# ortk95/planetmapper

Hardware: NVIDIA B200
Metric: full-backplane Mpix/s (FP64) + mapped-cube voxels/s at 1-8 B200 vs host CPU (higher is better)
Workload: dtype f64

## Files before the change

planetmapper_b200/csrc/backplane_kernels.cu:

```cuda
#include "pm_device.cuh"
#include "pm_kernels.h"

#include <cstdlib>

namespace pm {

constexpr int kPerThread = 4;
#ifndef PM_IMG_PARAM_CTAS
#define PM_IMG_PARAM_CTAS 4
#endif
constexpr int kImgParamCtas = PM_IMG_PARAM_CTAS;

__device__ __forceinline__ int slot(uint64_t mask, int k) { return __popcll(mask & (bit(k) - 1ull)); }

struct PlaneOffsets {
    int64_t byte_off[PM_N_PLANES];
    int64_t frame_stride;
};
static PlaneOffsets make_plane_offsets(uint64_t mask, int64_t plane_stride) {
    PlaneOffsets po;
    int slot = 0;
    for (int k = 0; k < PM_N_PLANES; k++) {
        po.byte_off[k] = (int64_t)slot * plane_stride * (int64_t)sizeof(double);
        if (mask & bit(k)) slot++;
    }
    po.frame_stride = (int64_t)slot * plane_stride;
    return po;
}

struct PlaneSink {
    char *base;
    const PlaneOffsets &po;
    __device__ __forceinline__ void put(int k, double v) const {
        __stcs(reinterpret_cast<double *>(base + po.byte_off[k]), v);
    }
};

template <bool kSky, uint64_t kFixedMask>
__device__ __forceinline__ void img_tile(const FrameD &fs, uint32_t tile, uint32_t nx, uint32_t npx, int per_thread,
                                         uint64_t mask, const PlaneOffsets &po, double *__restrict__ out) {
    uint32_t idx = tile * (uint32_t)(kBlock * per_thread) + threadIdx.x;
    uint32_t yi = idx / nx, xi = idx - yi * nx;
#pragma unroll 1
    for (int r = 0; r < per_thread && idx < npx; r++) {
        PlaneSink sink{reinterpret_cast<char *>(out + idx), po};
        image_pixel<kSky, kFixedMask>(fs, (double)xi, (double)yi, mask, sink);
        idx += kBlock;
        xi += kBlock;
        while (xi >= nx) {
            xi -= nx;
            yi++;
        }
    }
}

template <bool kSky, uint64_t kFixedMask>
__global__ void __launch_bounds__(kBlock, 4) backplanes_img_kernel(const PMFrame *__restrict__ frames, uint32_t nx,
                                                                   uint32_t npx, int per_thread, uint64_t mask,
                                                                   const __grid_constant__ PlaneOffsets po,
                                                                   double *__restrict__ out_all) {
    __shared__ FrameD fs;
    load_frame(fs, frames + blockIdx.y);
    img_tile<kSky, kFixedMask>(fs, blockIdx.x, nx, npx, per_thread, mask, po,
                               out_all + (int64_t)blockIdx.y * __popcll(mask) * npx);
}

__device__ __forceinline__ uint32_t centre_out_tile(uint32_t k, uint32_t n_tiles, uint32_t centre) {
    const uint32_t lo = centre, hi = n_tiles - 1u - centre;
    const uint32_t j = (k + 1u) >> 1;
    if (j <= min(lo, hi)) return (k & 1u) ? centre + j : centre - j;
    return lo < hi ? k : n_tiles - 1u - k;
}
template <bool kSky, uint64_t kFixedMask>
__global__ void __launch_bounds__(kBlock, kImgParamCtas) backplanes_img_param_kernel(
    const __grid_constant__ FrameD fs, uint32_t nx, uint32_t npx, int per_thread, uint32_t centre_tile, uint64_t mask,
    const __grid_constant__ PlaneOffsets po, double *__restrict__ out) {
    img_tile<kSky, kFixedMask>(fs, centre_out_tile(blockIdx.x, gridDim.x, centre_tile), nx, npx, per_thread, mask,
                               po, out);
}

template <bool kSky, bool kRingAll>
__global__ void __launch_bounds__(kBlock, 4) backplanes_points_param_kernel(const __grid_constant__ FrameD fs,
                                                                            const double *__restrict__ x_in,
                                                                            const double *__restrict__ y_in,
                                                                            int64_t n, uint64_t mask,
                                                                            const __grid_constant__ PlaneOffsets po,
                                                                            double *__restrict__ out) {
    const int64_t first = (int64_t)blockIdx.x * (kBlock * kPerThread) + threadIdx.x;
#pragma unroll 1
    for (int r = 0; r < kPerThread; r++) {
        const int64_t idx = first + r * kBlock;
        if (idx >= n) break;
        PlaneSink sink{reinterpret_cast<char *>(out + idx), po};
        image_point<kSky, kRingAll>(fs, __ldg(x_in + idx), __ldg(y_in + idx), mask, sink);
    }
}

constexpr uint64_t kXYMapMask = bit(PM_PIXEL_X) | bit(PM_PIXEL_Y);

template <uint64_t kFixedMask>
__device__ __forceinline__ void map_tile(const FrameD &fs, const double *__restrict__ lon_in,
                                         const double *__restrict__ lat_in, int64_t n, uint64_t mask,
                                         const PlaneOffsets &po, double *__restrict__ out) {
    const int64_t first = (int64_t)blockIdx.x * (kBlock * kPerThread) + threadIdx.x;
#pragma unroll 1
    for (int r = 0; r < kPerThread; r++) {
        const int64_t idx = first + r * kBlock;
        if (idx >= n) break;
        PlaneSink sink{reinterpret_cast<char *>(out + idx), po};
        map_cell<kFixedMask>(fs, __ldg(lon_in + idx), __ldg(lat_in + idx), mask, sink);
    }
}

template <uint64_t kFixedMask>
__global__ void __launch_bounds__(kBlock, 4) backplanes_map_kernel(const PMFrame *__restrict__ frame,
                                                                   const double *__restrict__ lon_in,
                                                                   const double *__restrict__ lat_in,
                                                                   int64_t n, uint64_t mask,
                                                                   const __grid_constant__ PlaneOffsets po,
                                                                   double *__restrict__ out) {
    __shared__ FrameD fs;
    load_frame(fs, frame + blockIdx.y);
    map_tile<kFixedMask>(fs, lon_in, lat_in, n, mask, po, out + (int64_t)blockIdx.y * po.frame_stride);
}

template <uint64_t kFixedMask>
__global__ void __launch_bounds__(kBlock, 4) backplanes_map_param_kernel(const __grid_constant__ FrameD fs,
// ... 148 lines not shown
    return (unsigned)(blocks < 1 ? 1 : blocks);
}

constexpr uint64_t kDefaultStackMask = kLonLatMask | kCentricMask | kIllumMask | kStateMask;

static int pick_per_thread(int64_t n, int64_t n_batches, int sm_count, int ctas_per_sm) {
    const int64_t tiles = ((n + kBlock - 1) / kBlock) * n_batches;
    const int64_t target = (int64_t)sm_count * ctas_per_sm * 3;
    int per = 16;
    while (per > 1 && tiles / per < target) per >>= 1;
    return per;
}

cudaError_t launch_backplanes_img(const PMFrame *frames, int n_frames, int nx, int ny, uint64_t mask,
                                  double *out, int sm_count, cudaStream_t st) {
    const int64_t npx = (int64_t)nx * ny;
    if (npx >= (1ll << 31)) return cudaErrorInvalidValue;
    const PlaneOffsets po = make_plane_offsets(mask, npx);
    static const int forced = tune_int("PM_IMG_PER_THREAD", 0);
    const int per = forced > 0 ? forced : pick_per_thread(npx, n_frames, sm_count, 4);
    const int64_t chunk = (int64_t)kBlock * per;
    dim3 grid((unsigned)((npx + chunk - 1) / chunk), n_frames);
    static const bool no_fixed = tune_int("PM_IMG_NO_FIXED_MASK", 0) != 0;
    if (mask == kDefaultStackMask && !no_fixed)
        backplanes_img_kernel<false, kDefaultStackMask><<<grid, kBlock, 0, st>>>(frames, (uint32_t)nx, (uint32_t)npx,
                                                                                   per, mask, po, out);
    else if (mask & kSkyMask)
        backplanes_img_kernel<true, 0><<<grid, kBlock, 0, st>>>(frames, (uint32_t)nx, (uint32_t)npx, per, mask, po, out);
    else
        backplanes_img_kernel<false, 0><<<grid, kBlock, 0, st>>>(frames, (uint32_t)nx, (uint32_t)npx, per, mask, po, out);
    count_launches(1);
    return cudaGetLastError();
}
cudaError_t launch_backplanes_img_host(const PMFrame *frame_host, int nx, int ny, uint64_t mask, double *out,
                                       int sm_count, cudaStream_t st) {
    const int64_t npx = (int64_t)nx * ny;
    if (npx >= (1ll << 31)) return cudaErrorInvalidValue;
    FrameD fs;
    load_frame_host(fs, frame_host);
    const PlaneOffsets po = make_plane_offsets(mask, npx);
    static const int forced = tune_int("PM_IMG_PER_THREAD", 0);
    const int per = forced > 0 ? forced : pick_per_thread(npx, 1, sm_count, kImgParamCtas);
    const int64_t chunk = (int64_t)kBlock * per;
    const int64_t n_tiles = (npx + chunk - 1) / chunk;
    dim3 grid((unsigned)n_tiles, 1);
    double cy = frame_host->y0 < 0.0 ? 0.0 : (frame_host->y0 > ny - 1.0 ? ny - 1.0 : frame_host->y0);
    double cx = frame_host->x0 < 0.0 ? 0.0 : (frame_host->x0 > nx - 1.0 ? nx - 1.0 : frame_host->x0);
    if (!(cy == cy) || !(cx == cx)) cy = cx = 0.0;
    int64_t ct = ((int64_t)cy * nx + (int64_t)cx) / chunk;
    static const bool linear = tune_int("PM_IMG_ORDER", 1) == 0;
    if (linear) ct = 0;
    const uint32_t centre = (uint32_t)(ct < 0 ? 0 : (ct >= n_tiles ? n_tiles - 1 : ct));
    if (mask == kDefaultStackMask)
        backplanes_img_param_kernel<false, kDefaultStackMask><<<grid, kBlock, 0, st>>>(
            fs, (uint32_t)nx, (uint32_t)npx, per, centre, mask, po, out);
    else if (mask & kSkyMask)
        backplanes_img_param_kernel<true, 0><<<grid, kBlock, 0, st>>>(fs, (uint32_t)nx, (uint32_t)npx, per, centre, mask,
                                                                       po, out);
    else
        backplanes_img_param_kernel<false, 0><<<grid, kBlock, 0, st>>>(fs, (uint32_t)nx, (uint32_t)npx, per, centre, mask,
                                                                        po, out);
    count_launches(1);
    return cudaGetLastError();
}
cudaError_t launch_backplanes_points_host(const PMFrame *frame_host, const double *x, const double *y, int64_t n,
                                          uint64_t mask, uint32_t flags, double *out, cudaStream_t st) {
    FrameD fs;
    load_frame_host(fs, frame_host);
    const PlaneOffsets po = make_plane_offsets(mask, n);
    const unsigned grid = chunks_for(n);
    if (!(mask & kSkyMask))
        backplanes_points_param_kernel<false, false><<<grid, kBlock, 0, st>>>(fs, x, y, n, mask, po, out);
    else if (flags & PM_FLAG_RING_ALL)
        backplanes_points_param_kernel<true, true><<<grid, kBlock, 0, st>>>(fs, x, y, n, mask, po, out);
    else
        backplanes_points_param_kernel<true, false><<<grid, kBlock, 0, st>>>(fs, x, y, n, mask, po, out);
    count_launches(1);
    return cudaGetLastError();
}
cudaError_t launch_backplanes_map(const PMFrame *frames, int n_frames, const double *lon, const double *lat,
                                  int64_t n, uint64_t mask, double *out, int sm_count, cudaStream_t st) {
    (void)sm_count;
    const dim3 grid(chunks_for(n), (unsigned)n_frames);
    const PlaneOffsets po = make_plane_offsets(mask, n);
    if (mask == kXYMapMask)
        backplanes_map_kernel<kXYMapMask><<<grid, kBlock, 0, st>>>(frames, lon, lat, n, mask, po, out);
    else
        backplanes_map_kernel<0><<<grid, kBlock, 0, st>>>(frames, lon, lat, n, mask, po, out);
    count_launches(1);
    return cudaGetLastError();
}
cudaError_t launch_backplanes_map_host(const PMFrame *frame_host, const double *lon, const double *lat, int64_t n,
                                       uint64_t mask, double *out, int sm_count, cudaStream_t st) {
    (void)sm_count;
    FrameD fs;
    load_frame_host(fs, frame_host);
    const PlaneOffsets po = make_plane_offsets(mask, n);
    if (mask == kXYMapMask)
        backplanes_map_param_kernel<kXYMapMask><<<chunks_for(n), kBlock, 0, st>>>(fs, lon, lat, n, mask, po, out);
    else
        backplanes_map_param_kernel<0><<<chunks_for(n), kBlock, 0, st>>>(fs, lon, lat, n, mask, po, out);
    count_launches(1);
    return cudaGetLastError();
}
cudaError_t launch_xy2lonlat(const PMFrame *frame, const double *x, const double *y, int64_t n, double *lon,
                             double *lat, unsigned long long *n_missed, int sm_count, cudaStream_t st) {
    (void)sm_count;
    xy2lonlat_kernel<<<chunks_for(n), kBlock, 0, st>>>(frame, x, y, n, lon, lat, n_missed);
    count_launches(1);
// ... 39 lines not shown
```

planetmapper_b200/csrc/pm_device.cuh:

```cuda
#pragma once

#include "../../include/pm_b200.h"
#include "pm_math.cuh"

namespace pm {

struct V3 {
    double x, y, z;
};

PM_HD V3 mk(double x, double y, double z) { return V3{x, y, z}; }
PM_HD V3 operator+(V3 a, V3 b) { return mk(a.x + b.x, a.y + b.y, a.z + b.z); }
PM_HD V3 operator-(V3 a, V3 b) { return mk(a.x - b.x, a.y - b.y, a.z - b.z); }
PM_HD V3 operator-(V3 a) { return mk(-a.x, -a.y, -a.z); }
PM_HD V3 operator*(double s, V3 a) { return mk(s * a.x, s * a.y, s * a.z); }
PM_HD double dot(V3 a, V3 b) { return fma(a.x, b.x, fma(a.y, b.y, a.z * b.z)); }
PM_HD V3 cross(V3 a, V3 b) {
    return mk(fma(a.y, b.z, -a.z * b.y), fma(a.z, b.x, -a.x * b.z), fma(a.x, b.y, -a.y * b.x));
}
PM_HD V3 mul3(V3 a, const double *s) { return mk(a.x * s[0], a.y * s[1], a.z * s[2]); }
PM_HD V3 axpy(double s, V3 b, V3 a) { return mk(fma(s, b.x, a.x), fma(s, b.y, a.y), fma(s, b.z, a.z)); }
PM_HD double norm(V3 a) { return fast_sqrt_lite(dot(a, a)); }
PM_HD V3 ld3(const double *p) { return mk(p[0], p[1], p[2]); }
PM_HD bool finite3(V3 a) { return fabs(a.x) < INFINITY && fabs(a.y) < INFINITY && fabs(a.z) < INFINITY; }
PM_HD V3 mxv(const double *m, V3 v) {
    return mk(fma(m[0], v.x, fma(m[1], v.y, m[2] * v.z)), fma(m[3], v.x, fma(m[4], v.y, m[5] * v.z)),
              fma(m[6], v.x, fma(m[7], v.y, m[8] * v.z)));
}
PM_HD V3 mtxv(const double *m, V3 v) {
    return mk(fma(m[0], v.x, fma(m[3], v.y, m[6] * v.z)), fma(m[1], v.x, fma(m[4], v.y, m[7] * v.z)),
              fma(m[2], v.x, fma(m[5], v.y, m[8] * v.z)));
}
PM_HD_NOINLINE double pymod360_slow(double a) {
    double r = ::fmod(a, 360.0);
    if (r != 0.0 && r < 0.0) r += 360.0;
    return r;
}
PM_HD double pymod360(double a) { return (a >= 0.0 && a < 360.0) ? a : pymod360_slow(a); }

struct FrameD {
    PMFrame f;
    double inv_c;
    double inv_r[3];
    double nw[3];
    double k[3];
    double wn;
    double rp;
    double e2, ep2;
    double inv_omf2;
    double omf;
    double P0b[3], VTb[3], ATb[3], VOb[3], S0b[3], VSb[3];
    double G[9];
    double y0[3];
    double y0m2;
    double As[6];
    double inv_kmpa;
    int biaxial;
    int pad_;
};

constexpr int kDeriveItems = 13;

PM_HD double ex_mul(double a, double b) {
#ifdef __CUDA_ARCH__
    return __dmul_rn(a, b);
#else
    return a * b;
#endif
}
PM_HD double ex_add(double a, double b) {
#ifdef __CUDA_ARCH__
    return __dadd_rn(a, b);
#else
    return a + b;
#endif
}
PM_HD double ex_div(double a, double b) {
#ifdef __CUDA_ARCH__
    return __ddiv_rn(a, b);
#else
    return a / b;
#endif
}
PM_HD double ex_sqrt(double a) {
#ifdef __CUDA_ARCH__
    return __dsqrt_rn(a);
#else
    return ::sqrt(a);
#endif
}
PM_HD double ex_dot3(double a0, double b0, double a1, double b1, double a2, double b2) {
    return ex_add(ex_add(ex_mul(a0, b0), ex_mul(a1, b1)), ex_mul(a2, b2));
}

PM_HD void derive_frame_item(FrameD &s, int item) {
    const PMFrame &f = s.f;
    if (item >= 3 && item <= 8) {
        const double *src = item == 3 ? f.P0 : item == 4 ? f.VT : item == 5 ? f.AT : item == 6 ? f.VO : item == 7 ? f.S0 : f.VS;
        double *dst = item == 3 ? s.P0b : item == 4 ? s.VTb : item == 5 ? s.ATb : item == 6 ? s.VOb : item == 7 ? s.S0b : s.VSb;
        for (int r = 0; r < 3; r++)
            dst[r] = ex_dot3(f.R0[3 * r], src[0], f.R0[3 * r + 1], src[1], f.R0[3 * r + 2], src[2]);
        if (item == 3) {
            for (int r = 0; r < 3; r++) s.y0[r] = ex_mul(-dst[r], ex_div(1.0, f.radii[r]));
            s.y0m2 = fma(s.y0[0], s.y0[0], fma(s.y0[1], s.y0[1], ex_mul(s.y0[2], s.y0[2])));
        }
    } else if (item >= 9 && item <= 11) {
        const int r = item - 9;
        for (int c = 0; c < 3; c++)
            s.G[3 * r + c] = ex_dot3(f.R0[3 * r], f.M[3 * c], f.R0[3 * r + 1], f.M[3 * c + 1], f.R0[3 * r + 2], f.M[3 * c + 2]);
    } else if (item == 12) {
        const double sc = kRpd / 3600.0;
        for (int c = 0; c < 3; c++) {
            s.As[c] = -ex_mul(f.A[c], sc);
            s.As[3 + c] = ex_mul(f.A[3 + c], sc);
        }
        s.inv_kmpa = ex_div(1.0, f.km_per_arcsec);
    } else if (item == 0) {
        s.inv_c = ex_div(1.0, f.clight);
        const double w2 = ex_dot3(f.omega[0], f.omega[0], f.omega[1], f.omega[1], f.omega[2], f.omega[2]);
        const double wn = ex_sqrt(w2);
        s.wn = wn;
        s.k[0] = wn > 0.0 ? ex_div(f.omega[0], wn) : 0.0;
        s.k[1] = wn > 0.0 ? ex_div(f.omega[1], wn) : 0.0;
        s.k[2] = wn > 0.0 ? ex_div(f.omega[2], wn) : 0.0;
    } else if (item == 1) {
        const double a = f.radii[0], b = f.radii[1], c = f.radii[2];
        s.inv_r[0] = ex_div(1.0, a);
        s.inv_r[1] = ex_div(1.0, b);
        s.inv_r[2] = ex_div(1.0, c);
        const double m = fmin(a, fmin(b, c));
        const double ma = ex_div(m, a), mb = ex_div(m, b), mc = ex_div(m, c);
        s.nw[0] = ex_mul(ma, ma);
        s.nw[1] = ex_mul(mb, mb);
        s.nw[2] = ex_mul(mc, mc);
    } else if (item == 2) {
        const double rp = ex_add(f.re, -ex_mul(f.f, f.re));
        const double re2 = ex_mul(f.re, f.re), rp2 = ex_mul(rp, rp);
        const double omf = ex_add(1.0, -f.f);
        s.rp = rp;
        s.e2 = ex_add(1.0, -ex_div(rp2, re2));
        s.ep2 = ex_add(ex_div(re2, rp2), -1.0);
        s.omf = omf;
        s.inv_omf2 = ex_div(1.0, ex_mul(omf, omf));
        s.biaxial = (f.radii[0] == f.radii[1]) && (f.re == f.radii[0]) && (fabs(rp - f.radii[2]) <= 4e-16 * f.radii[2]);
        s.pad_ = 0;
    }
}

#ifdef __CUDACC__
__device__ __forceinline__ void load_frame(FrameD &s, const PMFrame *__restrict__ g) {
    const double *src = reinterpret_cast<const double *>(g);
    double *dst = reinterpret_cast<double *>(&s.f);
    for (int i = threadIdx.x; i < PM_FRAME_NDOUBLES; i += blockDim.x) dst[i] = __ldg(src + i);
    __syncthreads();
    const int w = threadIdx.x >> 5, l = threadIdx.x & 31;
    int item = -1;
    if (blockDim.x >= 128) {
        if (w == 0 && l < 6) item = 3 + l;
        else if (w == 1 && l < 4) item = 9 + l;
        else if (w == 2 && l < 2) item = l;
        else if (w == 3 && l == 0) item = 2;
    } else if (threadIdx.x < kDeriveItems) {
        item = threadIdx.x;
    }
    if (item >= 0) derive_frame_item(s, item);
    __syncthreads();
}
#endif
inline void load_frame_host(FrameD &s, const PMFrame *g) {
    s.f = *g;
    for (int i = 0; i < kDeriveItems; i++) derive_frame_item(s, i);
}

#ifndef PM_GRAZING_COS2
#define PM_GRAZING_COS2 3.0e-3
#endif
constexpr double kGrazingCos2 = PM_GRAZING_COS2;

// ... 38 lines not shown
    const V3 t = mk(fma(k.x, ku, -u.x), fma(k.y, ku, -u.y), fma(k.z, ku, -u.z));
    return axpy(r.omc, t, axpy(r.s, kxu, u));
}
PM_HD V3 spin_bwd(const FrameD &fs, Rot r, V3 u) { return spin_bwd_c(fs, r, u, cross(ld3(fs.k), u)); }
PM_HD V3 to_body(const FrameD &fs, Rot r, V3 v) { return spin_fwd(fs, r, mxv(fs.f.R0, v)); }
PM_HD V3 from_body(const FrameD &fs, Rot r, V3 u) { return mtxv(fs.f.R0, spin_bwd(fs, r, u)); }
PM_HD V3 target_pos_b(const FrameD &fs, double dt) {
    const double h = 0.5 * dt * dt;
    return mk(fma(fs.ATb[0], h, fma(fs.VTb[0], dt, fs.P0b[0])), fma(fs.ATb[1], h, fma(fs.VTb[1], dt, fs.P0b[1])),
              fma(fs.ATb[2], h, fma(fs.VTb[2], dt, fs.P0b[2])));
}

PM_HD void recrad_angles(V3 v, double &ra, double &dec) {
    dec = fast_atan2_xpos(v.z, fast_sqrt(fma(v.x, v.x, v.y * v.y)));
    double lon = fast_atan2(v.y, v.x);
    if (lon < 0.0) lon += kTwoPi;
    ra = lon;
}
PM_HD V3 radrec1(double ra, double dec) {
    double sr, cr, sd, cd;
    sincos_full(ra, sr, cr);
    sincos_full(dec, sd, cd);
    return mk(cr * cd, sr * cd, sd);
}
PM_HD double vsep(V3 a, V3 b) { return fast_atan2_ypos(norm(cross(a, b)), dot(a, b)); }

struct RayHit {
    V3 pp;
    double ixx;
    double a;
    double t;
    double cos2;
};
PM_HD bool surfpt_y(const FrameD &fs, V3 y, double ym2, V3 u, V3 &p, RayHit &hit) {
    const V3 x = mul3(u, fs.inv_r);
    const double xx = dot(x, x), yx = dot(y, x);
    if (!(xx > 0.0)) return false;
    const double ixx = fast_rcp(xx);
    const double a = -(yx * ixx);
    const V3 pp = axpy(a, x, y);
    const double pm2 = dot(pp, pp);
    if (!(pm2 < INFINITY)) return false;
    hit.pp = pp;
    hit.ixx = ixx;
    hit.a = a;
    hit.cos2 = 1.0 - pm2;
    double h;
    if (ym2 > 1.0) {
        if (pm2 > 1.0) return false;
        if (yx > 0.0) return false;
        h = -fast_sqrt_lite((1.0 - pm2) * ixx);
    } else if (ym2 == 1.0) {
        h = -a;
    } else {
        h = fast_sqrt_lite(fmax(0.0, 1.0 - pm2) * ixx);
    }
    hit.t = a + h;
    p = mul3(axpy(h, x, pp), fs.f.radii);
    return true;
}
PM_HD bool surfpt(const FrameD &fs, V3 o, V3 u, V3 &p, RayHit &hit) {
    const V3 y = mul3(o, fs.inv_r);
    return surfpt_y(fs, y, dot(y, y), u, p, hit);
}

struct Intercept {
    V3 p;
    V3 u;
    Rot r;
    double dt;
    double L;
    double lt;
};

PM_HD_NOINLINE bool sincpt_converge(const FrameD &fs, V3 u0, double &dt, V3 &p, double &range) {
    const PMFrame &f = fs.f;
    for (int it = 0; it < 8; it++) {
        const Rot r = make_rot(fs, dt);
        const V3 o = spin_fwd(fs, r, -target_pos_b(fs, dt));
        RayHit hit;
        if (!surfpt(fs, o, spin_fwd(fs, r, u0), p, hit)) return false;
        range = hit.t;
        const double t = dt + f.t_ref;
        const double t_new = f.et - hit.t * fs.inv_c;
        if (!(fabs(t_new - t) > 1.0e-17 * fabs(t_new))) break;
        dt = t_new - f.t_ref;
    }
    return true;
}

PM_HD bool sincpt(const FrameD &fs, V3 u0, Intercept &it) {
    const PMFrame &f = fs.f;
    V3 p1, p2;
    RayHit h1, h2;
    if (!surfpt_y(fs, ld3(fs.y0), fs.y0m2, u0, p1, h1)) return false;
    const double lt1 = h1.t * fs.inv_c;

    const double dt1 = (f.et - lt1) - f.t_ref;
    const Rot r1 = make_rot(fs, dt1);
    if (!surfpt(fs, spin_fwd(fs, r1, -target_pos_b(fs, dt1)), spin_fwd(fs, r1, u0), p2, h2)) return false;
    const double lt2 = h2.t * fs.inv_c;

    double dt = (f.et - lt2) - f.t_ref;
    V3 p;
    double L;
    if (fabs(dt1) > PM_T(kPixC)[kPixDt1Min] && h2.cos2 > PM_T(kPixC)[kPixGrazing]) {
        const double lam = fast_div_lite(dt - dt1, dt1 - (dt - dt1));
        dt = fma(lam, dt1, dt1) + f.t_ref;
        dt -= f.t_ref;
        const V3 pps = axpy(lam, h2.pp - h1.pp, h2.pp);
        const double hs = fast_sqrt_lite(fmax(1.0 - dot(pps, pps), 0.0) * fma(lam, h2.ixx - h1.ixx, h2.ixx));
        L = fma(lam, h2.a - h1.a, h2.a) - hs;
        it.r = make_rot(fs, dt);
        it.u = spin_fwd(fs, it.r, u0);
        p = axpy(-hs, it.u, mul3(pps, fs.f.radii));
    } else {
        double dt_c = dt, L_c;
        V3 p_c;
        if (!sincpt_converge(fs, u0, dt_c, p_c, L_c)) return false;
        dt = dt_c;
        p = p_c;
        L = L_c;
        it.r = make_rot(fs, dt);
        it.u = spin_fwd(fs, it.r, u0);
    }
    it.p = p;
    it.dt = dt;
    it.L = L;
    it.lt = L * fs.inv_c;
    return true;
}

PM_HD void geodetic_general(const FrameD &fs, double rho, double z, double &lat, double &alt) {
    const PMFrame &f = fs.f;
    if (f.f == 0.0) {
        lat = fast_atan2_xpos(z, rho);
        alt = fast_sqrt(fma(rho, rho, z * z)) - f.re;
        return;
    }
    double sb = f.re * z, cb = fs.rp * rho;
    double n = fast_rsqrt(fma(sb, sb, cb * cb) + sqrt_guard());
    sb *= n;
    cb *= n;
    double num = z, den = rho;
#pragma unroll 1
    for (int i = 0; i < 8; i++) {
        num = fma(fs.ep2 * fs.rp, sb * sb * sb, z);
        den = fma(-fs.e2 * f.re, cb * cb * cb, rho);
        double nsb = fs.omf * num, ncb = den;
        n = fast_rsqrt(fma(nsb, nsb, ncb * ncb) + sqrt_guard());
        nsb *= n;
        ncb *= n;
        const double change = fabs(nsb - sb) + fabs(ncb - cb);
        sb = nsb;
        cb = ncb;
        if (change <= 4.0e-16) break;
    }
// ... 79 lines not shown
PM_HD_NOINLINE double doppler_factor_closed(double beta) { return fast_sqrt(fast_div(1.0 + beta, 1.0 - beta)); }
PM_HD_NOINLINE double light_time_rate_closed(double a, double b, double c) { return fast_div(a - b, c + a); }
PM_HD double doppler_factor(const FrameD &fs, double rv) {
    const double beta = rv * fs.inv_c;
    if (fabs(beta) < PM_T(kPixC)[kPixBetaMax])
        return fma(beta, fma(beta, fma(beta, fma(beta, fma(beta, 0.375, 0.375), 0.5), 0.5), 1.0), 1.0);
    return doppler_factor_closed(beta);
}

PM_HD double radial_velocity(const FrameD &fs, double a, double b) {
    const double ac = a * fs.inv_c;
    double dlt = (a - b) * fs.inv_c * fma(ac, ac - 1.0, 1.0);
    if (!(fabs(ac) < PM_T(kPixC)[kPixBetaMax])) dlt = light_time_rate_closed(a, b, fs.f.clight);
    return fma(-dlt, a, a) - b;
}

struct Illum {
    double phase, incdnc, emissn, azimuth;
};
PM_HD void illum_angles(V3 n, V3 s, V3 e, bool want_az, Illum &out) {
    const V3 cse = cross(s, e), cns = cross(n, s), cne = cross(n, e);
    const double dse = dot(s, e), dns = dot(n, s), dne = dot(n, e);
    const double mns = norm(cns), mne = norm(cne);
    out.phase = fast_atan2_ypos(norm(cse), dse);
    out.incdnc = fast_atan2_ypos(mns, dns);
    out.emissn = fast_atan2_ypos(mne, dne);
    if (want_az) {
        const double nn = dot(n, n);
        const double a = fma(dse, nn, -dne * dns);
        out.azimuth = fast_atan2_ypos(fast_sqrt_pos(nn) * fabs(dot(n, cse)), -a);
    }
}

PM_HD void illum_at(const FrameD &fs, V3 p, V3 p0 , V3 e, Rot r, double dt, bool want_az,
                    Illum &out) {
    const PMFrame &f = fs.f;
    const double h = 0.5 * dt * dt;
    const V3 base = mk(fs.S0b[0] - fma(fs.ATb[0], h, fma(fs.VTb[0], dt, p0.x)),
                       fs.S0b[1] - fma(fs.ATb[1], h, fma(fs.VTb[1], dt, p0.y)),
                       fs.S0b[2] - fma(fs.ATb[2], h, fma(fs.VTb[2], dt, p0.z)));
    const V3 VSb = ld3(fs.VSb);
    V3 sv = axpy(dt, VSb, base);
    const double lts = fast_sqrt_pos(dot(sv, sv)) * fs.inv_c;
    sv = axpy(dt - (lts - f.lts0), VSb, base);
    const V3 s_b = spin_fwd(fs, r, sv);
    const V3 n = mul3(p, fs.nw);
    illum_angles(n, s_b, e, want_az, out);
}

struct PointGeom {
    V3 p0;
    V3 X0;
    Rot r;
    double dt, L, lt;
};
PM_HD void point_geom(const FrameD &fs, V3 p, PointGeom &g) {
    const PMFrame &f = fs.f;
    double lt = norm(ld3(fs.P0b) + p) * fs.inv_c;
#pragma unroll 1
    for (int pass = 0; pass < 2; pass++) {
        const double dt = (f.et - lt) - f.t_ref;
        const Rot r = make_rot(fs, dt);
        const V3 p0 = spin_bwd(fs, r, p);
        const V3 X0 = target_pos_b(fs, dt) + p0;
        const double L = norm(X0);
        lt = L * fs.inv_c;
        g.p0 = p0;
        g.X0 = X0;
        g.r = r;
        g.dt = dt;
        g.L = L;
        g.lt = lt;
    }
}
PM_HD double point_rv(const FrameD &fs, V3 p, const PointGeom &g) {
    const double iL = fast_rcp(g.L);
    const V3 ph0 = iL * g.X0;
    const V3 vt = axpy(g.dt, ld3(fs.ATb), ld3(fs.VTb));
// ... 58 lines not shown

PM_HD void limb_coordinates(const FrameD &fs, V3 ov, double &lon_deg, double &lat_deg, double &dist) {
    const PMFrame &f = fs.f;
    lon_deg = lat_deg = dist = NAN;
    const double n2 = dot(ov, ov);
    if (!(n2 > 0.0)) return;
    const V3 u = fast_rsqrt(n2) * ov;
    const V3 P0 = ld3(f.P0);
    const V3 pn = dot(P0, u) * u;
    const double near_dist = norm(P0 - pn);
    const V3 tv = obsvec2targvec(fs, pn);
    const V3 x = mul3(tv, fs.inv_r);
    const double xn2 = dot(x, x);
    if (!(xn2 > 0.0)) return;
    const V3 sp = fast_rsqrt(xn2) * tv;
    double lon, lat, alt;
    recpgr(fs, sp, fs.biaxial != 0, lon, lat, alt);
    lon_deg = lon * kDpr;
    lat_deg = lat * kDpr;
    dist = near_dist - norm(sp);
}

PM_HD constexpr uint64_t bit(int k) { return 1ull << k; }
constexpr uint64_t kKmMask = bit(PM_KM_X) | bit(PM_KM_Y) | bit(PM_ANGULAR_X) | bit(PM_ANGULAR_Y);
constexpr uint64_t kLonLatMask = bit(PM_LON_GRAPHIC) | bit(PM_LAT_GRAPHIC) | bit(PM_LOCAL_SOLAR_TIME);
constexpr uint64_t kCentricMask = bit(PM_LON_CENTRIC) | bit(PM_LAT_CENTRIC);
constexpr uint64_t kIllumMask = bit(PM_PHASE) | bit(PM_INCIDENCE) | bit(PM_EMISSION) | bit(PM_AZIMUTH);
constexpr uint64_t kStateMask = bit(PM_DISTANCE) | bit(PM_RADIAL_VELOCITY) | bit(PM_DOPPLER);
constexpr uint64_t kLimbMask = bit(PM_LIMB_DISTANCE) | bit(PM_LIMB_LON_GRAPHIC) | bit(PM_LIMB_LAT_GRAPHIC);
constexpr uint64_t kRingMask = bit(PM_RING_RADIUS) | bit(PM_RING_LON_GRAPHIC) | bit(PM_RING_DISTANCE);
constexpr uint64_t kSurfMask = kLonLatMask | kCentricMask | kIllumMask | kStateMask | kRingMask;
constexpr uint64_t kSkyMask = bit(PM_RA) | bit(PM_DEC) | kKmMask | kLimbMask | kRingMask;

template <bool kSky, uint64_t kFixedMask = 0, bool kRingAll = false, class Sink>
PM_HD void image_pixel(const FrameD &fs, double x, double y, uint64_t mask_in, Sink &out) {
    const PMFrame &f = fs.f;
    const double nan = NAN;
    const uint64_t mask = kFixedMask ? kFixedMask : (kSky ? mask_in : (mask_in & ~kSkyMask));
    if (mask & bit(PM_PIXEL_X)) out.put(PM_PIXEL_X, x);
    if (mask & bit(PM_PIXEL_Y)) out.put(PM_PIXEL_Y, y);

    const double dx = x - f.x0, dy = y - f.y0;
    const bool try_disc = (mask & kSurfMask) && !(f.optimize_speed != 0.0 && fma(dx, dx, dy * dy) > f.r_cut2);
    V3 v = mk(nan, nan, nan);
    if (try_disc || (kSky && (mask & kSkyMask))) v = xy2ray_local(fs, x, y);
    V3 d2 = mk(nan, nan, nan);
    if (kSky && (mask & kSkyMask)) {
        const V3 d = mtxv(f.M, v);
        double ra, dec;
        recrad_angles(d, ra, dec);
        const double ra_deg = ra * kDpr, dec_deg = dec * kDpr;
        if (mask & bit(PM_RA)) out.put(PM_RA, ra_deg);
        if (mask & bit(PM_DEC)) out.put(PM_DEC, dec_deg);
        if (mask & (kKmMask | kLimbMask | kRingMask)) d2 = radrec1(ra_deg * kRpd, dec_deg * kRpd);
        if (mask & kKmMask) {
            double ax, ay;
            obsvec2angular(f, d2, ax, ay);
            const double kx = fma(f.ang2km[0], ax, f.ang2km[1] * ay);
            const double ky = fma(f.ang2km[2], ax, f.ang2km[3] * ay);
            if (mask & bit(PM_KM_X)) out.put(PM_KM_X, kx);
            if (mask & bit(PM_KM_Y)) out.put(PM_KM_Y, ky);
            if (mask & bit(PM_ANGULAR_X)) out.put(PM_ANGULAR_X, fast_div(kx, f.km_per_arcsec));
            if (mask & bit(PM_ANGULAR_Y)) out.put(PM_ANGULAR_Y, fast_div(ky, f.km_per_arcsec));
        }
    }

    bool on_disc = false;
    Intercept it;
    const V3 u0 = mxv(fs.G, v);
    if (try_disc) on_disc = sincpt(fs, u0, it);

    double v_dist = nan;
    if (on_disc) {
        const V3 p = it.p;
        if (mask & (kLonLatMask | kCentricMask)) {
            const double rho = fast_sqrt_lite(fma(p.x, p.x, p.y * p.y));
            const double lon_e = fast_atan2(p.y, p.x);
            if (mask & kLonLatMask) {
                double l = f.lon_sign * lon_e;
                if (l < 0.0) l += kTwoPi;
                const double v_lon = l * kDpr;
                double lat, alt;
                if (fs.biaxial) {
                    lat = fast_atan2_xpos(p.z * fs.inv_omf2, rho);
                } else {
                    geodetic_general(fs, rho, p.z, lat, alt);
                }
                if (mask & bit(PM_LON_GRAPHIC)) out.put(PM_LON_GRAPHIC, v_lon);
                if (mask & bit(PM_LAT_GRAPHIC)) out.put(PM_LAT_GRAPHIC, lat * kDpr);
                if (mask & bit(PM_LOCAL_SOLAR_TIME)) out.put(PM_LOCAL_SOLAR_TIME, local_solar_time(f, v_lon));
            }
            if (mask & bit(PM_LON_CENTRIC)) out.put(PM_LON_CENTRIC, lon_e * kDpr);
            if (mask & bit(PM_LAT_CENTRIC)) out.put(PM_LAT_CENTRIC, fast_atan2_xpos(p.z, rho) * kDpr);
        }
        if (mask & (kIllumMask | kStateMask | kRingMask)) {
            const V3 kxp = cross(ld3(fs.k), p);
            const V3 p0 = spin_bwd_c(fs, it.r, p, kxp);
            if (mask & kIllumMask) {
                Illum il;
                illum_at(fs, p, p0, -it.u, it.r, it.dt, (mask & bit(PM_AZIMUTH)) != 0, il);
                if (mask & bit(PM_PHASE)) out.put(PM_PHASE, il.phase * kDpr);
                if (mask & bit(PM_INCIDENCE)) out.put(PM_INCIDENCE, il.incdnc * kDpr);
                if (mask & bit(PM_EMISSION)) out.put(PM_EMISSION, il.emissn * kDpr);
                if (mask & bit(PM_AZIMUTH)) out.put(PM_AZIMUTH, il.azimuth * kDpr);
            }
            v_dist = it.lt * f.clight;
            if (mask & bit(PM_DISTANCE)) out.put(PM_DISTANCE, v_dist);
            if (mask & (bit(PM_RADIAL_VELOCITY) | bit(PM_DOPPLER))) {
                const V3 vt = axpy(it.dt, ld3(fs.ATb), ld3(fs.VTb));
                const double a = fma(fs.wn, dot(kxp, it.u), dot(vt, u0));
                const double b = dot(ld3(fs.VOb), u0);
                const double rv = radial_velocity(fs, a, b);
                if (mask & bit(PM_RADIAL_VELOCITY)) out.put(PM_RADIAL_VELOCITY, rv);
                if (mask & bit(PM_DOPPLER)) out.put(PM_DOPPLER, doppler_factor(fs, rv));
            }
        }
    } else {
        const uint64_t m = mask & (kLonLatMask | kCentricMask | kIllumMask | kStateMask);
#pragma unroll
        for (int k = 0; k <= PM_DOPPLER; k++)
            if ((kLonLatMask | kCentricMask | kIllumMask | kStateMask) & bit(k))
                if (m & bit(k)) out.put(k, nan);
    }

    if (kSky && (mask & kLimbMask)) {
        double llon, llat, ldist;
        limb_coordinates(fs, d2, llon, llat, ldist);
        if (mask & bit(PM_LIMB_DISTANCE)) out.put(PM_LIMB_DISTANCE, ldist);
        if (mask & bit(PM_LIMB_LON_GRAPHIC)) out.put(PM_LIMB_LON_GRAPHIC, llon);
        if (mask & bit(PM_LIMB_LAT_GRAPHIC)) out.put(PM_LIMB_LAT_GRAPHIC, llat);
    }
    if (kSky && (mask & kRingMask)) {
        double rad, rl, rd;
        ring_coordinates(fs, d2, rad, rl, rd);
        if (!kRingAll && rd > v_dist) rad = rl = rd = nan;
        if (mask & bit(PM_RING_RADIUS)) out.put(PM_RING_RADIUS, rad);
        if (mask & bit(PM_RING_LON_GRAPHIC)) out.put(PM_RING_LON_GRAPHIC, rl);
        if (mask & bit(PM_RING_DISTANCE)) out.put(PM_RING_DISTANCE, rd);
    }
}

template <bool kSky, bool kRingAll, class Sink>
PM_HD void image_point(const FrameD &fs, double x, double y, uint64_t mask_in, Sink &out) {
    if (fabs(x) < INFINITY && fabs(y) < INFINITY) {
        image_pixel<kSky, 0, kRingAll>(fs, x, y, mask_in, out);
        return;
    }
#pragma unroll 1
    for (int k = 0; k < PM_N_PLANES; k++)
        if (mask_in & bit(k)) out.put(k, k == PM_PIXEL_X ? x : (k == PM_PIXEL_Y ? y : (double)NAN));
}

template <uint64_t kFixedMask = 0, class Sink>
PM_HD void map_cell(const FrameD &fs, double lon_deg, double lat_deg, uint64_t mask_in, Sink &out) {
    const uint64_t mask = kFixedMask ? kFixedMask : mask_in;
    const PMFrame &f = fs.f;
    const double nan = NAN;
    const double lonm = (fabs(lon_deg) < INFINITY) ? pymod360(lon_deg) : nan;
    const double latm = (fabs(lat_deg) < INFINITY) ? lat_deg : nan;
    if (mask & bit(PM_LON_GRAPHIC)) out.put(PM_LON_GRAPHIC, lonm);
    if (mask & bit(PM_LAT_GRAPHIC)) out.put(PM_LAT_GRAPHIC, latm);
    const bool lon_ok = lonm == lonm;
    const bool ok = lon_ok && (latm == latm);
    if (mask & bit(PM_LOCAL_SOLAR_TIME))
        out.put(PM_LOCAL_SOLAR_TIME, lon_ok ? local_solar_time(f, lonm) : nan);

    double v_clon = nan, v_clat = nan, v_g = nan, v_i = nan, v_e = nan, v_az = nan, v_dist = nan, v_rv = nan,
           v_dop = nan, v_ra = nan, v_dec = nan, v_x = nan, v_y = nan, v_kx = nan, v_ky = nan, v_ax = nan,
           v_ay = nan;
    double limb_lon = nan, limb_lat = nan, limb_dist = nan, ring_rad = nan, ring_lon = nan, ring_dist = nan;
    if (ok) {
        const V3 tv = pgrrec0(fs, lonm * kRpd, latm * kRpd);
        if (mask & kCentricMask) {
            double lo, la;
            reclat_angles(tv, lo, la);
            v_clon = lo * kDpr;
            v_clat = la * kDpr;
        }
// ... 246 lines not shown
```

Measured before the change: 30270.

## Add spin-symmetric fast path skipping body rotations in surface intercept

Adds a per-frame flag, computed when frame data is derived, marking bodies that are axisymmetric about the spin axis with negligible light-time rotation shift. For such frames, templated kernel variants skip the rotation of the observer position and ray direction inside the light-time intercept iterations. They reuse the ray-scaled direction and its reciprocal across both surface solves, and compute illumination in the unrotated frame without rotating the sun vector or the intercept point back. This cuts FP64 arithmetic per pixel, at the cost of extra kernel instantiations and code size, and results within the stated tolerance of the shift threshold may differ slightly.

New measurement: 32750 (median of 6 runs). +8.2%, better.

```diff
diff --git a/planetmapper_b200/csrc/backplane_kernels.cu b/planetmapper_b200/csrc/backplane_kernels.cu
--- a/planetmapper_b200/csrc/backplane_kernels.cu
+++ b/planetmapper_b200/csrc/backplane_kernels.cu
@@ -36,7 +36,7 @@
     }
 };
 
-template <bool kSky, uint64_t kFixedMask>
+template <bool kSky, uint64_t kFixedMask, bool kSpinSym>
 __device__ __forceinline__ void img_tile(const FrameD &fs, uint32_t tile, uint32_t nx, uint32_t npx, int per_thread,
                                          uint64_t mask, const PlaneOffsets &po, double *__restrict__ out) {
     uint32_t idx = tile * (uint32_t)(kBlock * per_thread) + threadIdx.x;
@@ -44,7 +44,7 @@
 #pragma unroll 1
     for (int r = 0; r < per_thread && idx < npx; r++) {
         PlaneSink sink{reinterpret_cast<char *>(out + idx), po};
-        image_pixel<kSky, kFixedMask>(fs, (double)xi, (double)yi, mask, sink);
+        image_pixel<kSky, kFixedMask, false, kSpinSym>(fs, (double)xi, (double)yi, mask, sink);
         idx += kBlock;
         xi += kBlock;
         while (xi >= nx) {
@@ -61,8 +61,11 @@
                                                                    double *__restrict__ out_all) {
     __shared__ FrameD fs;
     load_frame(fs, frames + blockIdx.y);
-    img_tile<kSky, kFixedMask>(fs, blockIdx.x, nx, npx, per_thread, mask, po,
-                               out_all + (int64_t)blockIdx.y * __popcll(mask) * npx);
+    double *out = out_all + (int64_t)blockIdx.y * __popcll(mask) * npx;
+    if (fs.spin_sym)
+        img_tile<kSky, kFixedMask, true>(fs, blockIdx.x, nx, npx, per_thread, mask, po, out);
+    else
+        img_tile<kSky, kFixedMask, false>(fs, blockIdx.x, nx, npx, per_thread, mask, po, out);
 }
 
 __device__ __forceinline__ uint32_t centre_out_tile(uint32_t k, uint32_t n_tiles, uint32_t centre) {
@@ -71,15 +74,15 @@
     if (j <= min(lo, hi)) return (k & 1u) ? centre + j : centre - j;
     return lo < hi ? k : n_tiles - 1u - k;
 }
-template <bool kSky, uint64_t kFixedMask>
+template <bool kSky, uint64_t kFixedMask, bool kSpinSym>
 __global__ void __launch_bounds__(kBlock, kImgParamCtas) backplanes_img_param_kernel(
     const __grid_constant__ FrameD fs, uint32_t nx, uint32_t npx, int per_thread, uint32_t centre_tile, uint64_t mask,
     const __grid_constant__ PlaneOffsets po, double *__restrict__ out) {
-    img_tile<kSky, kFixedMask>(fs, centre_out_tile(blockIdx.x, gridDim.x, centre_tile), nx, npx, per_thread, mask,
-                               po, out);
-}
-
-template <bool kSky, bool kRingAll>
+    img_tile<kSky, kFixedMask, kSpinSym>(fs, centre_out_tile(blockIdx.x, gridDim.x, centre_tile), nx, npx, per_thread,
+                                         mask, po, out);
+}
+
+template <bool kSky, bool kRingAll, bool kSpinSym>
 __global__ void __launch_bounds__(kBlock, 4) backplanes_points_param_kernel(const __grid_constant__ FrameD fs,
                                                                             const double *__restrict__ x_in,
                                                                             const double *__restrict__ y_in,
@@ -92,7 +95,7 @@
         const int64_t idx = first + r * kBlock;
         if (idx >= n) break;
         PlaneSink sink{reinterpret_cast<char *>(out + idx), po};
-        image_point<kSky, kRingAll>(fs, __ldg(x_in + idx), __ldg(y_in + idx), mask, sink);
+        image_point<kSky, kRingAll, kSpinSym>(fs, __ldg(x_in + idx), __ldg(y_in + idx), mask, sink);
     }
 }
 
@@ -307,6 +310,17 @@
     count_launches(1);
     return cudaGetLastError();
 }
+template <bool kSpinSym>
+static void launch_img_param(const FrameD &fs, dim3 grid, uint32_t nx, uint32_t npx, int per, uint32_t centre,
+                             uint64_t mask, const PlaneOffsets &po, double *out, cudaStream_t st) {
+    if (mask == kDefaultStackMask)
+        backplanes_img_param_kernel<false, kDefaultStackMask, kSpinSym><<<grid, kBlock, 0, st>>>(fs, nx, npx, per, centre,
+                                                                                                mask, po, out);
+    else if (mask & kSkyMask)
+        backplanes_img_param_kernel<true, 0, kSpinSym><<<grid, kBlock, 0, st>>>(fs, nx, npx, per, centre, mask, po, out);
+    else
+        backplanes_img_param_kernel<false, 0, kSpinSym><<<grid, kBlock, 0, st>>>(fs, nx, npx, per, centre, mask, po, out);
+}
 cudaError_t launch_backplanes_img_host(const PMFrame *frame_host, int nx, int ny, uint64_t mask, double *out,
                                        int sm_count, cudaStream_t st) {
     const int64_t npx = (int64_t)nx * ny;
@@ -326,17 +340,22 @@
     static const bool linear = tune_int("PM_IMG_ORDER", 1) == 0;
     if (linear) ct = 0;
     const uint32_t centre = (uint32_t)(ct < 0 ? 0 : (ct >= n_tiles ? n_tiles - 1 : ct));
-    if (mask == kDefaultStackMask)
-        backplanes_img_param_kernel<false, kDefaultStackMask><<<grid, kBlock, 0, st>>>(
-            fs, (uint32_t)nx, (uint32_t)npx, per, centre, mask, po, out);
-    else if (mask & kSkyMask)
-        backplanes_img_param_kernel<true, 0><<<grid, kBlock, 0, st>>>(fs, (uint32_t)nx, (uint32_t)npx, per, centre, mask,
-                                                                       po, out);
-    else
-        backplanes_img_param_kernel<false, 0><<<grid, kBlock, 0, st>>>(fs, (uint32_t)nx, (uint32_t)npx, per, centre, mask,
-                                                                        po, out);
-    count_launches(1);
-    return cudaGetLastError();
+    if (fs.spin_sym)
+        launch_img_param<true>(fs, grid, (uint32_t)nx, (uint32_t)npx, per, centre, mask, po, out, st);
+    else
+        launch_img_param<false>(fs, grid, (uint32_t)nx, (uint32_t)npx, per, centre, mask, po, out, st);
+    count_launches(1);
+    return cudaGetLastError();
+}
+template <bool kSpinSym>
+static void launch_points_param(const FrameD &fs, unsigned grid, const double *x, const double *y, int64_t n,
+                                uint64_t mask, uint32_t flags, const PlaneOffsets &po, double *out, cudaStream_t st) {
+    if (!(mask & kSkyMask))
+        backplanes_points_param_kernel<false, false, kSpinSym><<<grid, kBlock, 0, st>>>(fs, x, y, n, mask, po, out);
+    else if (flags & PM_FLAG_RING_ALL)
+        backplanes_points_param_kernel<true, true, kSpinSym><<<grid, kBlock, 0, st>>>(fs, x, y, n, mask, po, out);
+    else
+        backplanes_points_param_kernel<true, false, kSpinSym><<<grid, kBlock, 0, st>>>(fs, x, y, n, mask, po, out);
 }
 cudaError_t launch_backplanes_points_host(const PMFrame *frame_host, const double *x, const double *y, int64_t n,
                                           uint64_t mask, uint32_t flags, double *out, cudaStream_t st) {
@@ -344,12 +363,10 @@
     load_frame_host(fs, frame_host);
     const PlaneOffsets po = make_plane_offsets(mask, n);
     const unsigned grid = chunks_for(n);
-    if (!(mask & kSkyMask))
-        backplanes_points_param_kernel<false, false><<<grid, kBlock, 0, st>>>(fs, x, y, n, mask, po, out);
-    else if (flags & PM_FLAG_RING_ALL)
-        backplanes_points_param_kernel<true, true><<<grid, kBlock, 0, st>>>(fs, x, y, n, mask, po, out);
-    else
-        backplanes_points_param_kernel<true, false><<<grid, kBlock, 0, st>>>(fs, x, y, n, mask, po, out);
+    if (fs.spin_sym)
+        launch_points_param<true>(fs, grid, x, y, n, mask, flags, po, out, st);
+    else
+        launch_points_param<false>(fs, grid, x, y, n, mask, flags, po, out, st);
     count_launches(1);
     return cudaGetLastError();
 }
diff --git a/planetmapper_b200/csrc/pm_device.cuh b/planetmapper_b200/csrc/pm_device.cuh
--- a/planetmapper_b200/csrc/pm_device.cuh
+++ b/planetmapper_b200/csrc/pm_device.cuh
@@ -56,7 +56,7 @@
     double As[6];
     double inv_kmpa;
     int biaxial;
-    int pad_;
+    int spin_sym;
 };
 
 constexpr int kDeriveItems = 13;
@@ -123,6 +123,10 @@
         s.k[0] = wn > 0.0 ? ex_div(f.omega[0], wn) : 0.0;
         s.k[1] = wn > 0.0 ? ex_div(f.omega[1], wn) : 0.0;
         s.k[2] = wn > 0.0 ? ex_div(f.omega[2], wn) : 0.0;
+        const double wperp = ex_sqrt(ex_add(ex_mul(f.omega[0], f.omega[0]), ex_mul(f.omega[1], f.omega[1])));
+        const double flat = fabs(ex_add(f.radii[0], -f.radii[2]));
+        const double shift = ex_mul(ex_mul(wperp, ex_div(ex_mul(2.0, f.radii[0]), f.clight)), flat);
+        s.spin_sym = (f.radii[0] == f.radii[1]) && (shift <= 1.0e-9);
     } else if (item == 1) {
         const double a = f.radii[0], b = f.radii[1], c = f.radii[2];
         s.inv_r[0] = ex_div(1.0, a);
@@ -143,7 +147,6 @@
         s.omf = omf;
         s.inv_omf2 = ex_div(1.0, ex_mul(omf, omf));
         s.biaxial = (f.radii[0] == f.radii[1]) && (f.re == f.radii[0]) && (fabs(rp - f.radii[2]) <= 4e-16 * f.radii[2]);
-        s.pad_ = 0;
     }
 }
 
@@ -248,11 +251,8 @@
     double t;
     double cos2;
 };
-PM_HD bool surfpt_y(const FrameD &fs, V3 y, double ym2, V3 u, V3 &p, RayHit &hit) {
-    const V3 x = mul3(u, fs.inv_r);
-    const double xx = dot(x, x), yx = dot(y, x);
-    if (!(xx > 0.0)) return false;
-    const double ixx = fast_rcp(xx);
+PM_HD bool surfpt_yx(const FrameD &fs, V3 y, double ym2, V3 x, double ixx, V3 &p, RayHit &hit) {
+    const double yx = dot(y, x);
     const double a = -(yx * ixx);
     const V3 pp = axpy(a, x, y);
     const double pm2 = dot(pp, pp);
@@ -275,6 +275,12 @@
     p = mul3(axpy(h, x, pp), fs.f.radii);
     return true;
 }
+PM_HD bool surfpt_y(const FrameD &fs, V3 y, double ym2, V3 u, V3 &p, RayHit &hit) {
+    const V3 x = mul3(u, fs.inv_r);
+    const double xx = dot(x, x);
+    if (!(xx > 0.0)) return false;
+    return surfpt_yx(fs, y, ym2, x, fast_rcp(xx), p, hit);
+}
 PM_HD bool surfpt(const FrameD &fs, V3 o, V3 u, V3 &p, RayHit &hit) {
     const V3 y = mul3(o, fs.inv_r);
     return surfpt_y(fs, y, dot(y, y), u, p, hit);
@@ -283,19 +289,25 @@
 struct Intercept {
     V3 p;
     V3 u;
+    V3 p0;
     Rot r;
     double dt;
     double L;
     double lt;
 };
 
+template <bool kSpinSym>
 PM_HD_NOINLINE bool sincpt_converge(const FrameD &fs, V3 u0, double &dt, V3 &p, double &range) {
     const PMFrame &f = fs.f;
     for (int it = 0; it < 8; it++) {
-        const Rot r = make_rot(fs, dt);
-        const V3 o = spin_fwd(fs, r, -target_pos_b(fs, dt));
+        V3 o = -target_pos_b(fs, dt), u = u0;
+        if (!kSpinSym) {
+            const Rot r = make_rot(fs, dt);
+            o = spin_fwd(fs, r, o);
+            u = spin_fwd(fs, r, u0);
+        }
         RayHit hit;
-        if (!surfpt(fs, o, spin_fwd(fs, r, u0), p, hit)) return false;
+        if (!surfpt(fs, o, u, p, hit)) return false;
         range = hit.t;
         const double t = dt + f.t_ref;
         const double t_new = f.et - hit.t * fs.inv_c;
@@ -305,16 +317,26 @@
     return true;
 }
 
+template <bool kSpinSym = false>
 PM_HD bool sincpt(const FrameD &fs, V3 u0, Intercept &it) {
     const PMFrame &f = fs.f;
     V3 p1, p2;
     RayHit h1, h2;
-    if (!surfpt_y(fs, ld3(fs.y0), fs.y0m2, u0, p1, h1)) return false;
+    const V3 x = mul3(u0, fs.inv_r);
+    const double xx = dot(x, x);
+    if (!(xx > 0.0)) return false;
+    const double ixx = fast_rcp(xx);
+    if (!surfpt_yx(fs, ld3(fs.y0), fs.y0m2, x, ixx, p1, h1)) return false;
     const double lt1 = h1.t * fs.inv_c;
 
     const double dt1 = (f.et - lt1) - f.t_ref;
-    const Rot r1 = make_rot(fs, dt1);
-    if (!surfpt(fs, spin_fwd(fs, r1, -target_pos_b(fs, dt1)), spin_fwd(fs, r1, u0), p2, h2)) return false;
+    if (kSpinSym) {
+        const V3 y2 = mul3(-target_pos_b(fs, dt1), fs.inv_r);
+        if (!surfpt_yx(fs, y2, dot(y2, y2), x, ixx, p2, h2)) return false;
+    } else {
+        const Rot r1 = make_rot(fs, dt1);
+        if (!surfpt(fs, spin_fwd(fs, r1, -target_pos_b(fs, dt1)), spin_fwd(fs, r1, u0), p2, h2)) return false;
+    }
     const double lt2 = h2.t * fs.inv_c;
 
     double dt = (f.et - lt2) - f.t_ref;
@@ -325,20 +347,31 @@
         dt = fma(lam, dt1, dt1) + f.t_ref;
         dt -= f.t_ref;
         const V3 pps = axpy(lam, h2.pp - h1.pp, h2.pp);
-        const double hs = fast_sqrt_lite(fmax(1.0 - dot(pps, pps), 0.0) * fma(lam, h2.ixx - h1.ixx, h2.ixx));
+        const double ixxs = kSpinSym ? ixx : fma(lam, h2.ixx - h1.ixx, h2.ixx);
+        const double hs = fast_sqrt_lite(fmax(1.0 - dot(pps, pps), 0.0) * ixxs);
         L = fma(lam, h2.a - h1.a, h2.a) - hs;
         it.r = make_rot(fs, dt);
-        it.u = spin_fwd(fs, it.r, u0);
-        p = axpy(-hs, it.u, mul3(pps, fs.f.radii));
+        if (kSpinSym) {
+            it.p0 = axpy(-hs, u0, mul3(pps, fs.f.radii));
+            p = spin_fwd(fs, it.r, it.p0);
+        } else {
+            it.u = spin_fwd(fs, it.r, u0);
+            p = axpy(-hs, it.u, mul3(pps, fs.f.radii));
+        }
     } else {
         double dt_c = dt, L_c;
         V3 p_c;
-        if (!sincpt_converge(fs, u0, dt_c, p_c, L_c)) return false;
+        if (!sincpt_converge<kSpinSym>(fs, u0, dt_c, p_c, L_c)) return false;
         dt = dt_c;
-        p = p_c;
         L = L_c;
         it.r = make_rot(fs, dt);
-        it.u = spin_fwd(fs, it.r, u0);
+        if (kSpinSym) {
+            it.p0 = p_c;
+            p = spin_fwd(fs, it.r, p_c);
+        } else {
+            p = p_c;
+            it.u = spin_fwd(fs, it.r, u0);
+        }
     }
     it.p = p;
     it.dt = dt;
@@ -484,18 +517,20 @@
     }
 }
 
-PM_HD void illum_at(const FrameD &fs, V3 p, V3 p0 , V3 e, Rot r, double dt, bool want_az,
-                    Illum &out) {
+PM_HD V3 sun_vec0(const FrameD &fs, V3 p0, double dt) {
     const PMFrame &f = fs.f;
     const double h = 0.5 * dt * dt;
     const V3 base = mk(fs.S0b[0] - fma(fs.ATb[0], h, fma(fs.VTb[0], dt, p0.x)),
                        fs.S0b[1] - fma(fs.ATb[1], h, fma(fs.VTb[1], dt, p0.y)),
                        fs.S0b[2] - fma(fs.ATb[2], h, fma(fs.VTb[2], dt, p0.z)));
     const V3 VSb = ld3(fs.VSb);
-    V3 sv = axpy(dt, VSb, base);
+    const V3 sv = axpy(dt, VSb, base);
     const double lts = fast_sqrt_pos(dot(sv, sv)) * fs.inv_c;
-    sv = axpy(dt - (lts - f.lts0), VSb, base);
-    const V3 s_b = spin_fwd(fs, r, sv);
+    return axpy(dt - (lts - f.lts0), VSb, base);
+}
+PM_HD void illum_at(const FrameD &fs, V3 p, V3 p0 , V3 e, Rot r, double dt, bool want_az,
+                    Illum &out) {
+    const V3 s_b = spin_fwd(fs, r, sun_vec0(fs, p0, dt));
     const V3 n = mul3(p, fs.nw);
     illum_angles(n, s_b, e, want_az, out);
 }
@@ -620,7 +655,7 @@
 constexpr uint64_t kSurfMask = kLonLatMask | kCentricMask | kIllumMask | kStateMask | kRingMask;
 constexpr uint64_t kSkyMask = bit(PM_RA) | bit(PM_DEC) | kKmMask | kLimbMask | kRingMask;
 
-template <bool kSky, uint64_t kFixedMask = 0, bool kRingAll = false, class Sink>
+template <bool kSky, uint64_t kFixedMask = 0, bool kRingAll = false, bool kSpinSym = false, class Sink>
 PM_HD void image_pixel(const FrameD &fs, double x, double y, uint64_t mask_in, Sink &out) {
     const PMFrame &f = fs.f;
     const double nan = NAN;
@@ -656,7 +691,7 @@
     bool on_disc = false;
     Intercept it;
     const V3 u0 = mxv(fs.G, v);
-    if (try_disc) on_disc = sincpt(fs, u0, it);
+    if (try_disc) on_disc = sincpt<kSpinSym>(fs, u0, it);
 
     double v_dist = nan;
     if (on_disc) {
@@ -682,11 +717,14 @@
             if (mask & bit(PM_LAT_CENTRIC)) out.put(PM_LAT_CENTRIC, fast_atan2_xpos(p.z, rho) * kDpr);
         }
         if (mask & (kIllumMask | kStateMask | kRingMask)) {
-            const V3 kxp = cross(ld3(fs.k), p);
-            const V3 p0 = spin_bwd_c(fs, it.r, p, kxp);
+            const V3 kxp = cross(ld3(fs.k), kSpinSym ? it.p0 : p);
+            const V3 p0 = kSpinSym ? it.p0 : spin_bwd_c(fs, it.r, p, kxp);
             if (mask & kIllumMask) {
                 Illum il;
-                illum_at(fs, p, p0, -it.u, it.r, it.dt, (mask & bit(PM_AZIMUTH)) != 0, il);
+                if (kSpinSym)
+                    illum_angles(mul3(p0, fs.nw), sun_vec0(fs, p0, it.dt), -u0, (mask & bit(PM_AZIMUTH)) != 0, il);
+                else
+                    illum_at(fs, p, p0, -it.u, it.r, it.dt, (mask & bit(PM_AZIMUTH)) != 0, il);
                 if (mask & bit(PM_PHASE)) out.put(PM_PHASE, il.phase * kDpr);
                 if (mask & bit(PM_INCIDENCE)) out.put(PM_INCIDENCE, il.incdnc * kDpr);
                 if (mask & bit(PM_EMISSION)) out.put(PM_EMISSION, il.emissn * kDpr);
@@ -696,7 +734,7 @@
             if (mask & bit(PM_DISTANCE)) out.put(PM_DISTANCE, v_dist);
             if (mask & (bit(PM_RADIAL_VELOCITY) | bit(PM_DOPPLER))) {
                 const V3 vt = axpy(it.dt, ld3(fs.ATb), ld3(fs.VTb));
-                const double a = fma(fs.wn, dot(kxp, it.u), dot(vt, u0));
+                const double a = fma(fs.wn, dot(kxp, kSpinSym ? u0 : it.u), dot(vt, u0));
                 const double b = dot(ld3(fs.VOb), u0);
                 const double rv = radial_velocity(fs, a, b);
                 if (mask & bit(PM_RADIAL_VELOCITY)) out.put(PM_RADIAL_VELOCITY, rv);
@@ -728,10 +766,10 @@
     }
 }
 
-template <bool kSky, bool kRingAll, class Sink>
+template <bool kSky, bool kRingAll, bool kSpinSym = false, class Sink>
 PM_HD void image_point(const FrameD &fs, double x, double y, uint64_t mask_in, Sink &out) {
     if (fabs(x) < INFINITY && fabs(y) < INFINITY) {
-        image_pixel<kSky, 0, kRingAll>(fs, x, y, mask_in, out);
+        image_pixel<kSky, 0, kRingAll, kSpinSym>(fs, x, y, mask_in, out);
         return;
     }
 #pragma unroll 1
```
